# HpWang-whu/YOHO

Hardware: AMD Instinct MI355X
Metric: keypoints/sec (5000 kp x60 rot desc+YOHO-O) (higher is better)
Workload: dtype fp16x2 split (2^-22-accurate products, fp32 accumulate); 1 GPU

## Files before the change

yoho_amd/csrc/api.hip:

```cpp
#include "common.h"
#include <cstdarg>
#include <cstdio>
#include <cstring>
#include <cstdlib>
#include <cmath>
#include <vector>

namespace yoho {

static thread_local char g_err[512] = "";

void set_error(const char* fmt, ...) {
    va_list ap;
    va_start(ap, fmt);
    vsnprintf(g_err, sizeof(g_err), fmt, ap);
    va_end(ap);
}

void clear_error() { g_err[0] = 0; }

int hip_fail(hipError_t e, const char* what, const char* file, int line) {
    set_error("HIP error %d (%s) at %s:%d: %s", (int)e, hipGetErrorString(e), file, line, what);
    return YOHO_EHIP;
}
// ... 307 lines not shown
                            if (g < 0) g = ug[2 * u];
                            int tap = 2 * tp + h;
                            if (tap >= NTAP) tap = 2 * tp;
                            slab4[(cfg * 7 + tp) * 32 + u] |= (g < 0 ? 0 : (int)N[g * NTAP + tap]) << (8 * (2 * gs + h));
                        }
        }
        if ((rc = upload_slot_tables16(slab4.data(), unitg.data(), c->tabs)) || (rc = gconv16_init())) { delete c; return rc; }
    }
    c->gconv_mode = 4;
    c->partII_mode = 2;
    {
        auto is = [](const char* name, const char* val) { const char* e = std::getenv(name); return e && std::strcmp(e, val) == 0; };
        auto num = [](const char* name) { const char* e = std::getenv(name); return e ? std::atoi(e) : 0; };
        c->env.partII_tail_staged = is("YOHO_PARTII_TAIL", "staged");
        c->env.transfer_staged = is("YOHO_TRANSFER", "staged");
        c->env.xf_steal = !is("YOHO_XF_STEAL", "0");
        c->env.nn_splits = num("YOHO_NN_SPLITS");
        c->env.fcgf_f32 = is("YOHO_FCGF", "f32");
        c->env.fcgf_full_maps = is("YOHO_FCGF_MAPS", "full");
        c->env.fcgf_norm_staged = is("YOHO_FCGF_NORM", "staged");
        c->env.fcgf_heads_staged = is("YOHO_FCGF_HEADS", "staged");
        if (const char* e = std::getenv("YOHO_WS_LIMIT_MB")) c->env.ws_limit_mb = std::atoll(e);
        if (is("YOHO_PARTII_L1", "3")) c->env.partII_l1_variant = FG_TILE256_W8;
    }
    if (const char* m = std::getenv("YOHO_FCGF_CELLS")) c->fcgf_cell_sort = std::atoi(m);
    if (const char* m = std::getenv("YOHO_FCGF_SORT")) c->fcgf_parity_sort = std::strcmp(m, "0") == 0 ? 0 : 1;
    if (const char* m = std::getenv("YOHO_FCGF_COORDS")) c->fcgf_hash_coords = std::strcmp(m, "hash") == 0 ? 1 : 0;
    if (const char* m = std::getenv("YOHO_NN")) c->nn_prefilter = std::strcmp(m, "brute") == 0 ? 0 : 1;
    if (const char* m = std::getenv("YOHO_PARTII")) c->partII_mode = std::strcmp(m, "f32") == 0 ? 0 : (std::strcmp(m, "fp16x2") == 0 ? 2 : (std::strcmp(m, "cgemm") == 0 ? 3 : (std::strcmp(m, "cgemm8") == 0 ? 4 : 1)));
    if (const char* m = std::getenv("YOHO_PARTI_CHUNK")) {
        int ck = 0, ns = 1;
        if (std::sscanf(m, "%dx%d", &ck, &ns) >= 1 && ck >= 0 && (ns == 1 || ns == 2)) { c->partI_chunk = (ck + 255) / 256 * 256; c->partI_streams = ns; }
    }
    if (const char* m = std::getenv("YOHO_GCONV")) c->gconv_mode = std::strcmp(m, "f32") == 0 ? 0 : (std::strcmp(m, "bf16x3") == 0 ? 1 : (std::strcmp(m, "fp16x2") == 0 ? 3 : (std::strcmp(m, "fgemm") == 0 ? 4 : (std::strcmp(m, "fgemm256") == 0 ? 5 : (std::strcmp(m, "fgemm128") == 0 ? 6 : (std::strcmp(m, "fgemm8") == 0 ? 7 : 2))))));
    c->fb = new FourierBasis();
    if ((rc = build_fourier(N, P, *c->fb))) { delete c->fb; delete c; return rc; }
    {
        std::vector<float> fpad(2 * 64 * 64, 0.f);
        for (int s = 0; s < G; ++s)
            for (int g = 0; g < G; ++g) {
                fpad[s * 64 + g] = (float)c->fb->F[s * G + g];
                fpad[64 * 64 + g * 64 + s] = (float)c->fb->F[s * G + g];
            }
        if ((rc = upload(fpad.data(), fpad.size() * sizeof(float), (void**)&c->dFpad)) || (rc = gft_init()) || (rc = fgemm_init()) || (rc = gft16_init())) { delete c->fb; delete c; return rc; }
        std::vector<unsigned short> f16;
        build_gft16_frags(*c->fb, f16);
        if ((rc = upload(f16.data(), f16.size() * sizeof(unsigned short), &c->dF16))) { delete c->fb; delete c; return rc; }
        hipDeviceProp_t prop;
        if (hipGetDeviceProperties(&prop, device) == hipSuccess && prop.multiProcessorCount > 0) c->nCU = prop.multiProcessorCount;
    }
    HIPCHK(hipMalloc((void**)&c->d_rflag, 4 * sizeof(int)));
    HIPCHK(hipMemset(c->d_rflag, 0, 4 * sizeof(int)));
// ... 89 lines not shown
    if ((rc = build_layer(c->p2[2], w->res_out, 512, 256, NTAP, nullptr))) return rc;
    if ((rc = build_layer(c->p2[3], w->fc0, 256, 512, 1, &w->fc0_bn))) return rc;
    if ((rc = build_layer(c->p2[4], w->fc1, 512, 128, 1, &w->fc1_bn))) return rc;
    if ((rc = build_layer(c->p2[5], w->fc2, 128, 4, 1, nullptr))) return rc;
    for (auto& L : c->p2) L.tabs = &c->tabs;
    c->has_partII = true;
    return 0;
}

int yoho_set_gconv_mode(yoho_ctx* c, int mode) {
    if (!c || mode < 0 || mode > 7) { set_error("yoho_set_gconv_mode: mode must be 0 (fp32 MFMA), 1 (bf16x3 MFMA), 2 (group-Fourier fp32 MFMA), 3 (fp16x2 MFMA), 4 (group-Fourier irrep GEMMs, fp16x2 MFMA), 5 or 6 (4 with the other two GEMM blockings), 7 (4 with fp8 correction products)"); return YOHO_EINVAL; }
    c->gconv_mode = mode;
    return 0;
}

int yoho_set_partI_schedule(yoho_ctx* c, int chunk_kp, int streams) {
    if (!c || chunk_kp < 0 || streams < 1 || streams > 2) { set_error("yoho_set_partI_schedule: chunk_kp >= 0 and streams 1 or 2"); return YOHO_EINVAL; }
    c->partI_chunk = (chunk_kp + 255) / 256 * 256;
    c->partI_streams = streams;
    return 0;
}

int yoho_set_partII_mode(yoho_ctx* c, int mode) {
    if (!c || mode < 0 || mode > 4) { set_error("yoho_set_partII_mode: mode must be 0 (fp32 MFMA), 1 (bf16x3), 2 (fp16x2 MFMA, direct cone kernels), 3 (fp16x2, 13-element cone layer as an implicit GEMM) or 4 (3 with fp8 correction products)"); return YOHO_EINVAL; }
    c->partII_mode = mode;
    return 0;
}

int yoho_set_nn_prefilter(yoho_ctx* c, int enable) {
    if (!c) { set_error("yoho_set_nn_prefilter: null ctx"); return YOHO_EINVAL; }
    c->nn_prefilter = enable ? 1 : 0;
    return 0;
}

int yoho_set_fcgf_sort(yoho_ctx* c, int parity_sort, int cell_sort) {
    if (!c) { set_error("yoho_set_fcgf_sort: null ctx"); return YOHO_EINVAL; }
    c->fcgf_parity_sort = parity_sort ? 1 : 0;
    c->fcgf_hash_coords = (cell_sort >= 0 && (cell_sort & 4)) ? 1 : 0;
    cell_sort = cell_sort < 0 ? 0 : (cell_sort & 3);
    c->fcgf_cell_sort = cell_sort > 2 ? 2 : cell_sort;
    return 0;
}

int yoho_set_nn_grid(yoho_ctx* c, double cell) {
    if (!c || !(cell >= 0.0) || !std::isfinite(cell)) { set_error("yoho_set_nn_grid: cell must be a finite number >= 0 (0 = brute force)"); return YOHO_EINVAL; }
    c->nn_cell = cell;
    return 0;
// ... 353 lines not shown
                            inv_np ? inv_np + (size_t)b0 * F : nullptr, s);
        if (rc) return rc;
    }
    return 0;
}

int yoho_group_mean_np(yoho_ctx* c, const float* eqv, int B, float* out, void* stream) {
    if (!c || !eqv || !out || B < 0) { set_error("yoho_group_mean_np: bad argument"); return YOHO_EINVAL; }
    if (B == 0) return 0;
    YOHO_NEED_ALIGNED("yoho_group_mean_np", 15, eqv, out);
    HIPCHK(hipSetDevice(c->device));
    return launch_group_mean_np(eqv, B, out, (hipStream_t)stream);
}

static bool partII_fourier_head(const yoho_ctx* c) {
    return c->partII_mode >= 2 && c->p2[0].wpg;
}

static int partII_pass16(yoho_ctx* c, const float* s0, const float* s1, const float* s2, const float* s3, const int64_t* idx,
                         int M, float* quat, hipStream_t s, int npl, const int64_t* const* ridx = nullptr, int istride = 1) {
    const int nT16 = (M + 15) / 16, nT = (M + TILE - 1) / TILE;
    const size_t ch16 = (size_t)npl * 15360;
    const size_t n128 = (size_t)nT * 16, n256 = (size_t)nT * 32, n512 = (size_t)nT * 64, n32 = (size_t)nT * 4;
    const size_t szG = c->partII_mode >= 3 ? (size_t)((nT + 7) / 8) * c->cone_nslot * 8 * 32768 : 0;
    const size_t szX = (size_t)nT16 * 16 * ch16, szA0 = std::max((size_t)nT16 * 32 * ch16, szG);
    const size_t szA1p = npl == 2 ? (size_t)nT16 * 64 * ch16 : 0;
    int rc;
    int* rf = c->d_rflag + 1;
    if (ridx && !partII_fourier_head(c)) { set_error("indexed PartII needs the default (fp16x2, Fourier first layer) mode"); return YOHO_EINVAL; }
    const bool fourier_head = npl == 2 && partII_fourier_head(c);
    const int kppad = (M + 255) / 256 * 256;
    char *bX = nullptr, *bA0 = nullptr, *bA1p = nullptr, *bP = nullptr;
    float *bH0 = nullptr, *bA1 = nullptr, *bF = nullptr, *bF0 = nullptr, *bF1 = nullptr, *bQ = nullptr, *bC = nullptr;
    if ((rc = bind_ws(c, s, [&](Arena& ar) {
            bX = ar.take<char>(szX);
            bA0 = ar.take<char>(szA0);
            bA1p = ar.take<char>(szA1p);
            bH0 = ar.take<float>(n256 * CHUNK_FLOATS);
            bA1 = ar.take<float>(n512 * CHUNK_FLOATS);
            bF = ar.take<float>(n256 * CHUNK_FLOATS);
            bF0 = ar.take<float>(n512 * CHUNK_FLOATS);
            bF1 = ar.take<float>(n128 * CHUNK_FLOATS);
            bQ = ar.take<float>(n32 * CHUNK_FLOATS);
            if (fourier_head) {
                bP = ar.take<char>(fgemm_planes_bytes(kppad, 128));
                bC = ar.take<float>(n256 * CHUNK_FLOATS);
            }
        }))) return rc;
    if (fourier_head) {
        if ((rc = launch_head2(s0, s1, s2, s3, idx, c->dP, c->p2_init_bn_s, c->p2_init_bn_t, M, nT, bP, kppad, c->dF16, s, ridx, istride, rf))) return rc;
        if ((rc = launch_fgemm(c->p2[0], bP, kppad, nT, nullptr, bC, 0, s, rf, c->env.partII_l1_variant))) return rc;
        if (c->partII_mode >= 3 && c->p2[1].wcg && !c->env.partII_tail_staged && mlp_head_supported(c->p2[3], c->p2[4], c->p2[5])) {
            const int nslot = c->cone_nslot;
            unsigned* amax = nullptr;
            if (c->partII_mode == 4) {
                amax = c->d_amax + 8;
                HIPCHK(hipMemsetAsync(amax, 0, sizeof(unsigned), s));
            }
            if ((rc = launch_gft16_invg(bC, bH0, bA0, c->cone_slot_of, nslot, c->dF16, c->p2[0].bn_s, c->p2[0].bn_t, nT, 32, c->nCU, s, rf, amax))) return rc;
            if ((rc = launch_cgemm(c->p2[1], bA0, nslot, c->cone_slot, c->cone_outg, nT, nT16, bA1p, s, rf, amax))) return rc;
            int n0[NTAP];
            for (int k = 0; k < NTAP; ++k) n0[k] = c->hN[k];
            if ((rc = launch_cone1(c->p2[2], bA1p, nT, nT16, nullptr, nullptr, n0, s, bF0))) return rc;
            return launch_mlp_head(c->p2[3], c->p2[4], c->p2[5], nullptr, nT, M, quat, s, bF0, &c->p2[2], bH0);
        }
        if ((rc = launch_gft16_invp(bC, bH0, bA0, nT16, c->dF16, c->p2[0].bn_s, c->p2[0].bn_t, nT, 32, c->nCU, s, rf))) return rc;
    } else {
        if ((rc = launch_pack16_partII(s0, s1, s2, s3, idx, c->dP, c->p2_init_bn_s, c->p2_init_bn_t, M, nT16, bX, s, npl, rf))) return rc;
        if ((rc = launch_gconv16(c->p2[0], bX, nT16, nullptr, nullptr, bA0, EPI_RAW32 | EPI_ACT, s, 1, bH0, nullptr, npl, rf))) return rc;
    }
    if (npl == 2) {
        int n0[NTAP];
        for (int k = 0; k < NTAP; ++k) n0[k] = c->hN[k];
        if ((rc = launch_gconv16(c->p2[1], bA0, nT16, nullptr, nullptr, bA1p, EPI_ACT, s, 2, nullptr, nullptr, npl, rf))) return rc;
        if (!c->env.partII_tail_staged && mlp_head_supported(c->p2[3], c->p2[4], c->p2[5])) {
            if ((rc = launch_cone1(c->p2[2], bA1p, nT, nT16, nullptr, nullptr, n0, s, bF0))) return rc;
            return launch_mlp_head(c->p2[3], c->p2[4], c->p2[5], nullptr, nT, M, quat, s, bF0, &c->p2[2], bH0);
        }
        if ((rc = launch_cone1(c->p2[2], bA1p, nT, nT16, bH0, bF, n0, s))) return rc;
    } else {
        if ((rc = launch_gconv16(c->p2[1], bA0, nT16, nullptr, nullptr, nullptr, EPI_ACT32, s, 2, nullptr, bA1, npl))) return rc;
        if ((rc = launch_gconv(conv_args(c->p2[2], bA1, nT, bH0, bF, nullptr, true), -1, EPI_RES | EPI_RAW, s))) return rc;
    }
// ... 262 lines not shown
```

yoho_amd/csrc/common.h:

```cpp
#pragma once
#include <hip/hip_runtime.h>
#include <stdint.h>
#include <stddef.h>
#include <initializer_list>
#include "yoho_hip.h"
#include "arena.h"

namespace yoho {

constexpr int G = 60;
constexpr int NTAP = 13;
constexpr int F = 32;
constexpr int TILE = 32;
constexpr int SLAB_FLOATS = 2 * TILE * 4;
constexpr int CHUNK_FLOATS = G * SLAB_FLOATS;

void set_error(const char* fmt, ...);
void clear_error();
inline bool yoho_misaligned(std::initializer_list<const void*> ps, unsigned mask) {
    for (const void* p : ps) if ((reinterpret_cast<uintptr_t>(p) & mask) != 0) return true;
    return false;
}
#define YOHO_NEED_ALIGNED(fn, mask, ...)                                                                                  \
    do {                                                                                                                  \
// ... 90 lines not shown
int launch_finalize_partI(const float* y, const float* x, int B, float* eqv, float* inv, float* inv_np, int layout16, hipStream_t s,
                          const float* x1 = nullptr, int B0 = 0);
struct FourierBasis {
    double rho[5][60][25];
    double F[60 * 60];
    int n0[13];
};
int build_fourier(const uint8_t* N, const uint8_t* P, FourierBasis& fb);
}
#include <vector>
#include <cstdlib>
namespace yoho {
void pack_fourier_weights(const FourierBasis& fb, const float* W, int cin, int cout, int cout_pad, std::vector<float>& out);
int gft_init();
int fgemm_init();
size_t fgemm_planes_bytes(int kppad, int cin);
void fgemm_qinfo(int* qi);
void fgemm_plane_offsets(int kppad, int cin, long long* off);
int pack_fgemm_weights(const FourierBasis& fb, const float* W, int cin, int cout, std::vector<unsigned short>& out, float* descale,
                       std::vector<unsigned short>* out8 = nullptr);
int pack_cgemm_weights(const float* W, int cin, int cout, int ntaps, std::vector<unsigned short>& out, float* descale, std::vector<unsigned short>& out8);
int cgemm_init();
int launch_cgemm(const Layer& L, const char* Bstages, int nslot, const unsigned char* slot, const unsigned char* outg, int nT32, int nTiles16,
                 char* out, hipStream_t s, int* rflag, const unsigned* amax);
int launch_gft16_invg(const float* in, float* res0, char* planesG, const int* slot_of, int nslot, const void* Ffrag, const float* bn_s,
                      const float* bn_t, int nTiles, int C8, int nCU, hipStream_t s, int* rflag, unsigned* amax);
int launch_fgemm(const Layer& L, const char* Bplanes, int kppad, int nT32, const float* res, float* out, int flags, hipStream_t s,
                 int* rflag = nullptr, FGemmBlocking blocking = FG_TILE128, const unsigned* amax = nullptr);
void build_gft16_frags(const FourierBasis& fb, std::vector<unsigned short>& out);
int gconv_layer(yoho_ctx* c, const float* x, int B, int cin, int cout, const float* W, const float* bias, int transpose, float* y,
                hipStream_t s);
int bn_stats(const float* x, int B, int C, float* mean, float* var, hipStream_t s);
int bn_relu_apply(const float* x, int B, int C, const float* scale, const float* shift, float* y, hipStream_t s);
int bn_relu_apply_sub(const float* x, int B, int C, const float* mean, const float* scale, const float* beta, float* y, hipStream_t s);
int bn_relu_backward(const float* x, const float* y, const float* dy, int B, int C, const float* gamma, const float* mean, const float* rstd,
                     int batch_stats, float* dx, float* dgamma, float* dbeta, hipStream_t s);
int gconv_wgrad(yoho_ctx* c, const float* x, const float* dy, int B, int cin, int cout, float* dW, float* db, hipStream_t s);
struct FcgfNet;
int fcgf_load(FcgfNet** out, const yoho_fcgf_config* cfg, const float* const* t, int ntensors, bool f32_kernels);
void fcgf_free(FcgfNet* n);
int fcgf_forward(yoho_ctx* ctx, const FcgfNet* net, const int* coords0, int n0, const int* off_host, int nb, float* out, hipStream_t s);
int fcgf_voxelize(yoho_ctx* ctx, const double* pts, int n, const double* R_host, double voxel, int64_t* sel, int* coords, float* pts_sel,
                  int* count_host, hipStream_t s);
int fcgf_rotate_select(const double* pts, const double* R_host, const int64_t* sel, int m, float* out, hipStream_t s);
int fcgf_voxelize_batch(yoho_ctx* ctx, const double* pts, int n, const double* R_host, int nb, double voxel, int64_t* sel, int* coords,
                        float* pts_sel, int* counts_host, hipStream_t s);
int launch_cone1(const Layer& L, const char* X, int nTiles32, int nTiles16, const float* res, float* out, const int* n0, hipStream_t s, float* part = nullptr);
// ... 74 lines not shown
    bool on = false;
    std::vector<hipEvent_t> pool;
    size_t used = 0;
    struct Span { int cat; hipEvent_t a, b; };
    std::vector<Span> spans;
    int open_cat = -1;
    hipEvent_t open_ev = nullptr;
    double flops[NCAT] = {0};
    double launches[NCAT] = {0};
};

}

struct yoho_env_switches {
    bool partII_tail_staged = false;
    bool transfer_staged = false;
    bool xf_steal = true;
    int nn_splits = 0;
    bool fcgf_f32 = false;
    bool fcgf_full_maps = false;
    bool fcgf_norm_staged = false;
    bool fcgf_heads_staged = false;
    yoho::FGemmBlocking partII_l1_variant = yoho::FG_TILE128;
    long long ws_limit_mb = 0;
};

struct yoho_ctx {
    int device = 0;
    yoho_env_switches env;
    float* dR32 = nullptr;
    double* dR64 = nullptr;
    int* dN = nullptr;
    int* dP = nullptr;
    unsigned* dPq = nullptr;
    uint8_t hN[60 * 13];
    uint8_t hP[60 * 60];
    float hR[60 * 9];
    bool has_partI = false, has_partII = false;
    yoho::Layer p1[4];
    yoho::Layer p2[6];
    float *p2_init_bn_s = nullptr, *p2_init_bn_t = nullptr;
    int partII_mode = 2;
    int cone_nslot = 0;
    int cone_slot_of[60];
    unsigned char cone_slot[13 * 13];
    unsigned char cone_outg[13];
// ... 73 lines not shown
```

yoho_amd/csrc/gemmf2.hip:

```cpp
#include <hip/hip_runtime.h>
#include <cstdlib>
#include <cstring>
#include "common.h"
#include "gemmf.h"

namespace yoho {

constexpr int F2_BUF = 24576;
constexpr int F2_LDS = 3 * F2_BUF;
constexpr int F3_BUF = 32768;
constexpr int F3_LDS = 3 * F3_BUF;

struct Frags2 {
    uintx4 ah[4], al[4], bh[2], bl[2];
};

template <int LO, int R>
__device__ __forceinline__ void read_frag2(const char* pa, const char* pb, Frags2& f) {
    if constexpr (R < 4) f.al[R] = *reinterpret_cast<const uintx4*>(pa + 8192 + R * 512);
    else if constexpr (R < 6) f.bh[R - 4] = *reinterpret_cast<const uintx4*>(pb + (R - 4) * 512);
    else if constexpr (R < 10) f.ah[R - 6] = *reinterpret_cast<const uintx4*>(pa + (R - 6) * 512);
    else f.bl[R - 10] = *reinterpret_cast<const uintx4*>(pb + LO + (R - 10) * 512);
}
template <int LO>
// ... 115 lines not shown
    constexpr std::false_type nodma;
    while (s + 4 < KT) {
        run(dma, P, Q);
        run(dma, Q, P);
    }
    if (KT >= 4) {
        run(dma, P, Q);
        run(nodma, Q, P);
    }
    run(nodma, P, Q);
    step(nodma, Q, P, smem + cur + lane_a, smem + cur + lane_b, nullptr, nullptr, nullptr);
}

template <int BUF, typename Dma>
__device__ __forceinline__ void ring_pipelined_idle(int KT, Dma&& dma) {
    __builtin_amdgcn_s_barrier();
    for (int s = 0; s + 1 < KT; ++s) {
        if (s + 3 < KT) dma(s + 3, (s % 3) * BUF);
        asm volatile("s_waitcnt vmcnt(0)" ::: "memory");
        __builtin_amdgcn_s_barrier();
    }
}

__global__ __launch_bounds__(256, 2) void fgemm2_kernel(FGemmArgs a, int flags) {
    extern __shared__ __attribute__((aligned(16))) char smem[];
    const int tid = threadIdx.x, lane = tid & 63;
    const int w = __builtin_amdgcn_readfirstlane(tid >> 6);
    int t = 0, local = 0, r = 0;
    if (!fg2_map(a, blockIdx.x & 7, blockIdx.x >> 3, (flags & F2_MIX) == 0, t, local, r)) return;
    const int d = a.dim[t];
    const int MT = a.MT[t], KS = d * a.cin / 32, KT = 2 * KS;
    const int nh = local & 1, pair = local >> 1;
    const int cg = pair / MT, mtile = pair - cg * MT;
    const int ntile = r + 8 * cg;
    const char* Ag = a.A + a.a_off[t] + (size_t)mtile * KS * FG_STAGE;
    const char* Bg = a.B + a.b_off[t] + (size_t)ntile * KS * FG_STAGE + nh * 2048;
    const int wm = w >> 1, wn = w & 1;
    const Dma2 dm(w, lane);
    const int lane_a = (lane >> 5) * 4096 + (wm * 128 + (lane & 31)) * 16;
    const int lane_b = 16384 + (lane >> 5) * 2048 + (wn * 64 + (lane & 31)) * 16;

    floatx16 acc[4][2];
    zero_acc(acc);
    auto dma = [&](int st, int buf) { dma_step(dm, Ag + step_off(st), Bg + step_off(st), smem + buf); };
    ring_prologue<F2_BUF>(KT, dma);
    const int row0 = mtile * 256 + wm * 128, colbase = ntile * 256 + nh * 128 + wn * 64;
    const bool rows_live = row0 < d * a.cout;
    const int jidx = colbase / a.kppad, kp0 = colbase - jidx * a.kppad, qbase = a.qbase[t];
    if ((flags & EPI_RES) && rows_live) residual_start(acc, row0, kp0, jidx, d, qbase, a.res, a.descale, a.cout, a.nT32, lane);
    asm volatile("s_waitcnt vmcnt(0)" ::: "memory");
    __builtin_amdgcn_s_barrier();
    if (!rows_live) return ring_pipelined_idle<F2_BUF>(KT, dma);

    Frags2 P;
    read_frags2<Dma2::LO>(smem + lane_a, smem + lane_b, P);
    ring_pipelined<F2_BUF, 6>(smem, Ag, Bg, KT, lane_a, lane_b, P,
        [&](auto dmac, const Frags2& f, Frags2& nf, const char* ra, const char* rb, const char* srcA, const char* srcB, char* buf) {
            step2<decltype(dmac)::value>(dm, f, acc, ra, rb, nf, srcA, srcB, buf);
        });
    coef_epilogue(acc, row0, kp0, jidx, d, qbase, a.out, a.bias, a.descale, a.cout, a.nT32, a.rflag, lane, flags);
}

struct Wave3 {
    int wm, wn, nh, lane_a, lane_b;
    Dma3 dm;
    __device__ __forceinline__ Wave3(int w8, int lane) : wm((w8 & 3) >> 1), wn(w8 & 1), nh(w8 >> 2), dm(w8, lane) {
        lane_a = (lane >> 5) * 4096 + (wm * 128 + (lane & 31)) * 16;
        lane_b = 16384 + (lane >> 5) * 4096 + (nh * 128 + wn * 64 + (lane & 31)) * 16;
    }
};

__global__ __launch_bounds__(512, 2) void fgemm3_kernel(FGemmArgs a, int flags) {
    extern __shared__ __attribute__((aligned(16))) char smem[];
    const int tid = threadIdx.x, lane = tid & 63;
    const Wave3 wv(__builtin_amdgcn_readfirstlane(tid >> 6), lane);
    int t = 0, local = 0, r = 0;
    if (!fg3_map(a, blockIdx.x & 7, blockIdx.x >> 3, t, local, r)) return;
    const int d = a.dim[t];
    const int MT = a.MT[t], KS = d * a.cin / 32, KT = 2 * KS;
    const int cg = local / MT, mtile = local - cg * MT;
    const int ntile = r + 8 * cg;
    const char* Ag = a.A + a.a_off[t] + (size_t)mtile * KS * FG_STAGE;
    const char* Bg = a.B + a.b_off[t] + (size_t)ntile * KS * FG_STAGE;

    floatx16 acc[4][2];
    zero_acc(acc);
    auto dma = [&](int st, int buf) { dma_step(wv.dm, Ag + step_off(st), Bg + step_off(st), smem + buf); };
    ring_prologue<F3_BUF>(KT, dma);
    const int row0 = mtile * 256 + wv.wm * 128, colbase = ntile * 256 + wv.nh * 128 + wv.wn * 64;
    const bool rows_live = row0 < d * a.cout;
    const int jidx = colbase / a.kppad, kp0 = colbase - jidx * a.kppad, qbase = a.qbase[t];
// ... 48 lines not shown
__device__ __forceinline__ void step3c(const Frags2& f, floatx16 (&acc)[4][2], Frags8& c8, const C8Scales& sc) {
#pragma unroll
    for (int i = 0; i < 4; ++i)
#pragma unroll
        for (int j = 0; j < 2; ++j) acc[i][j] = mfma_h(f.ah[i], f.bh[j], acc[i][j]);
#pragma unroll
    for (int i = 0; i < 4; ++i)
#pragma unroll
        for (int e = 0; e < 4; ++e) c8.a[i][4 * PAR + e] = (int)f.al[i][e];
#pragma unroll
    for (int j = 0; j < 2; ++j) {
        const Int2 l = frag_to_fp8(f.bl[j], sc.bl), h = frag_to_fp8(f.bh[j], sc.bh);
        c8.b[j][4 * PAR] = l.x; c8.b[j][4 * PAR + 1] = l.y; c8.b[j][4 * PAR + 2] = h.x; c8.b[j][4 * PAR + 3] = h.y;
    }
    if constexpr (PAR == 1) {
#pragma unroll
        for (int i = 0; i < 4; ++i)
#pragma unroll
            for (int j = 0; j < 2; ++j)
                acc[i][j] = __builtin_amdgcn_mfma_scale_f32_32x32x64_f8f6f4(c8.a[i], c8.b[j], acc[i][j], 0, 0, 0, 127 + 2 - 11, 0, sc.mfma_b);
    }
}

template <bool FP8, typename BSrc>
__device__ __forceinline__ void ring_plain(floatx16 (&acc)[4][2], char* smem, const Wave3& wv, const char* Ag, BSrc&& bsrc, int KT, bool rows_live,
                                           const C8Scales& sc) {
    Frags8 c8;
    if constexpr (FP8) {
#pragma unroll
        for (int i = 0; i < 4; ++i)
#pragma unroll
            for (int e = 0; e < 8; ++e) c8.a[i][e] = 0;
#pragma unroll
        for (int j = 0; j < 2; ++j)
#pragma unroll
            for (int e = 0; e < 8; ++e) c8.b[j][e] = 0;
    }
    int cur = 0, stg = 2 * F3_BUF;
    int s = 0;
    auto stage = [&] {
        const int s2 = s + 2 < KT ? s + 2 : KT - 1;
        dma_step(wv.dm, uniform_ptr(Ag + step_off(s2)), uniform_ptr(bsrc(s2)), smem + stg);
    };
    auto rotate = [&] { stg = cur; cur = cur == 2 * F3_BUF ? 0 : cur + F3_BUF; ++s; };
    auto one_step = [&](auto parity) {
        asm volatile("s_waitcnt vmcnt(4) lgkmcnt(0)" ::: "memory");
        __builtin_amdgcn_s_barrier();
        __builtin_amdgcn_sched_barrier(0);
        stage();
        Frags2 f;
        read_frags2<Dma3::LO>(smem + cur + wv.lane_a, smem + cur + wv.lane_b, f);
        if constexpr (FP8) step3c<decltype(parity)::value>(f, acc, c8, sc);
        else {
#pragma unroll
            for (int i = 0; i < 4; ++i)
#pragma unroll
                for (int j = 0; j < 2; ++j) acc[i][j] = mfma_h(f.al[i], f.bh[j], acc[i][j]);
#pragma unroll
            for (int i = 0; i < 4; ++i)
#pragma unroll
                for (int j = 0; j < 2; ++j) acc[i][j] = mfma_h(f.ah[i], f.bl[j], acc[i][j]);
#pragma unroll
            for (int i = 0; i < 4; ++i)
#pragma unroll
                for (int j = 0; j < 2; ++j) acc[i][j] = mfma_h(f.ah[i], f.bh[j], acc[i][j]);
        }
        rotate();
    };
    if (rows_live) {
        for (int it = 0; it < KT; it += 2) {
            one_step(std::integral_constant<int, 0>{});
            one_step(std::integral_constant<int, 1>{});
        }
    } else {
        for (int it = 0; it < KT; ++it) {
            asm volatile("s_waitcnt vmcnt(4) lgkmcnt(0)" ::: "memory");
            __builtin_amdgcn_s_barrier();
            stage();
            rotate();
        }
    }
    asm volatile("s_waitcnt vmcnt(0)" ::: "memory");
}

__global__ __launch_bounds__(512, 2) void fgemm3c_kernel(FGemmArgs a, int flags) {
    extern __shared__ __attribute__((aligned(16))) char smem[];
    const int tid = threadIdx.x, lane = tid & 63;
    const Wave3 wv(__builtin_amdgcn_readfirstlane(tid >> 6), lane);
    int t = 0, local = 0, r = 0;
    if (!fg3_map(a, blockIdx.x & 7, blockIdx.x >> 3, t, local, r)) return;
    const int d = a.dim[t];
    const int MT = a.MT[t], KS = d * a.cin / 32, KT = 2 * KS;
    const int cg = local / MT, mtile = local - cg * MT;
    const int ntile = r + 8 * cg;
    const char* Ag = a.A + a.a_off[t] + (size_t)mtile * KS * FG_STAGE;
    const char* Bg = a.B + a.b_off[t] + (size_t)ntile * KS * FG_STAGE;

    floatx16 acc[4][2];
    zero_acc(acc);
// ... 17 lines not shown
    const float* bias;
    const float* bn_s;
    const float* bn_t;
    char* out;
    int NTm, MT, KSt, ntap, nj, nslot, c8out, nT32, nTiles16;
    float descale;
    int* rflag;
    const unsigned* amax;
    unsigned char slot[13 * 13];
    unsigned char outg[16];
};

__device__ __forceinline__ void cg_split_pair(float x0, float x1, unsigned& hi, unsigned& lo) {
    typedef float f2 __attribute__((ext_vector_type(2)));
    f2 x;
    x.x = x0; x.y = x1;
    const halfx2 h = __builtin_convertvector(x, halfx2);
    const f2 r = x - __builtin_convertvector(h, f2);
    const halfx2 l = __builtin_convertvector(r, halfx2);
    __builtin_memcpy(&hi, &h, 4);
    __builtin_memcpy(&lo, &l, 4);
}

template <bool FP8>
__global__ __launch_bounds__(512, 2) void cgemm_kernel(CGemmArgs a) {
    extern __shared__ __attribute__((aligned(16))) char smem[];
    __shared__ int tapoff[16];
    const int tid = threadIdx.x, lane = tid & 63;
    const Wave3 wv(__builtin_amdgcn_readfirstlane(tid >> 6), lane);
    const int xcd = blockIdx.x & 7, slot_ = blockIdx.x >> 3;
    const int ct = xcd + 8 * (slot_ / a.MT), mtile = slot_ % a.MT;
    if (ct >= a.nj * a.NTm) return;
    const int j = ct / a.NTm, mt = ct - j * a.NTm;
    const int SPT = 2 * a.KSt;
    const int KT = a.ntap * SPT;
    if (tid < 16) tapoff[tid] = tid < a.ntap ? (int)a.slot[j * 13 + tid] : 0;
    const char* Ag = a.A + (size_t)mtile * (KT / 2) * FG_STAGE;
    const char* Bt = a.B + (size_t)mt * a.nslot * a.KSt * FG_STAGE;
    __syncthreads();
    auto bsrc = [&](int s) -> const char* {
        const int tap = s / SPT, within = s - tap * SPT;
        const int sl = __builtin_amdgcn_readfirstlane(tapoff[tap]);
        return Bt + (size_t)sl * a.KSt * FG_STAGE + step_off(within);
    };

    floatx16 acc[4][2];
    zero_acc(acc);
    C8Scales sc;
    if constexpr (FP8) sc = C8Scales(a.amax);
    dma_step(wv.dm, Ag, uniform_ptr(bsrc(0)), smem);
    dma_step(wv.dm, Ag + step_off(1), uniform_ptr(bsrc(1)), smem + F3_BUF);
    asm volatile("s_waitcnt vmcnt(0)" ::: "memory");
    __builtin_amdgcn_s_barrier();

    ring_plain<FP8>(acc, smem, wv, Ag, bsrc, KT, true, sc);

    const int half = lane >> 5, c32 = lane & 31;
    const int g = a.outg[j];
    unsigned top = 0u;
#pragma unroll
    for (int bi = 0; bi < 2; ++bi) {
        const int m = mt * 256 + wv.nh * 128 + wv.wn * 64 + bi * 32 + c32;
        if ((m >> 5) >= a.nT32 || (m >> 4) >= a.nTiles16) continue;
#pragma unroll
        for (int ai = 0; ai < 4; ++ai) {
#pragma unroll
            for (int q4 = 0; q4 < 4; ++q4) {
                const int o = mtile * 256 + wv.wm * 128 + ai * 32 + q4 * 8 + half * 4;
                const floatx4 b4 = *reinterpret_cast<const floatx4*>(a.bias + o);
                const floatx4 s4 = *reinterpret_cast<const floatx4*>(a.bn_s + o);
                const floatx4 t4 = *reinterpret_cast<const floatx4*>(a.bn_t + o);
                float y[4];
#pragma unroll
                for (int e = 0; e < 4; ++e) {
                    const float v = acc[ai][bi][4 * q4 + e] * a.descale + b4[e];
                    y[e] = fmaxf(v * s4[e] + t4[e], 0.f) * H2_ASCALE;
                    top = max(top, __float_as_uint(y[e]) & 0x7FFFFFFFu);
                }
                unsigned h0, l0, h1, l1;
                cg_split_pair(y[0], y[1], h0, l0);
                cg_split_pair(y[2], y[3], h1, l1);
                char* dst = a.out + (((size_t)(m >> 4) * a.c8out + (o >> 3)) * 2) * 15360 + g * 256 + (m & 15) * 16 + half * 8;
                *reinterpret_cast<uint2*>(dst) = uint2{h0, h1};
                *reinterpret_cast<uint2*>(dst + 15360) = uint2{l0, l1};
            }
        }
    }
    note_range_bits(a.rflag, top, FP16_MAX);
}

int cgemm_init() {
    HIPCHK(hipFuncSetAttribute(reinterpret_cast<const void*>(&cgemm_kernel<true>), hipFuncAttributeMaxDynamicSharedMemorySize, F3_LDS));
    HIPCHK(hipFuncSetAttribute(reinterpret_cast<const void*>(&cgemm_kernel<false>), hipFuncAttributeMaxDynamicSharedMemorySize, F3_LDS));
    return 0;
}

int launch_cgemm(const Layer& L, const char* Bstages, int nslot, const unsigned char* slot, const unsigned char* outg, int nT32, int nTiles16,
                 char* out, hipStream_t s, int* rflag, const unsigned* amax) {
    const bool fp8 = amax != nullptr;
    if (!(fp8 ? L.wcg8 : L.wcg) || L.cin % 32 || L.cout % 256) { set_error("cgemm: needs the cone-GEMM weight pack, cin %% 32 == 0, cout %% 256 == 0"); return YOHO_EINVAL; }
    if (nT32 == 0) return 0;
    CGemmArgs a;
    a.A = reinterpret_cast<const char*>(fp8 ? L.wcg8 : L.wcg); a.B = Bstages; a.bias = L.bias; a.bn_s = L.bn_s; a.bn_t = L.bn_t; a.out = out;
    a.NTm = (nT32 + 7) / 8; a.MT = L.cout / 256; a.KSt = L.cin / 32; a.ntap = 13; a.nj = 13; a.nslot = nslot; a.c8out = L.cout / 8;
    a.nT32 = nT32; a.nTiles16 = nTiles16; a.descale = L.wcg_descale; a.rflag = rflag; a.amax = amax;
    std::memcpy(a.slot, slot, 169);
    std::memset(a.outg, 0, 16);
    std::memcpy(a.outg, outg, 13);
    const int CT = a.nj * a.NTm;
    const int grid = 8 * ((CT + 7) / 8) * a.MT;
    if (fp8) hipLaunchKernelGGL(cgemm_kernel<true>, dim3(grid), dim3(512), F3_LDS, s, a);
    else hipLaunchKernelGGL(cgemm_kernel<false>, dim3(grid), dim3(512), F3_LDS, s, a);
    HIPCHK(hipGetLastError());
    return 0;
}

struct Frags3s {
    uintx4 ah[5], al[5], bh, bl;
};

template <int R>
__device__ __forceinline__ void read_frag3s(const char* pa, const char* pb, Frags3s& f) {
    if constexpr (R < 5) f.al[R] = *reinterpret_cast<const uintx4*>(pa + 8192 + R * 512);
    else if constexpr (R == 5) f.bh = *reinterpret_cast<const uintx4*>(pb);
    else if constexpr (R < 11) f.ah[R - 6] = *reinterpret_cast<const uintx4*>(pa + (R - 6) * 512);
    else f.bl = *reinterpret_cast<const uintx4*>(pb + 8192);
}

template <bool DMA, int D>
__device__ __forceinline__ void step3s(const Frags3s& f, floatx16 (&acc)[5][1], const char* ra, const char* rb, Frags3s& nf,
                                       const char* srcA, const char* srcB, char* dmabuf, const Dma3& dm) {
    sfor<0, 5>([&](auto gc) {
        constexpr int g = decltype(gc)::value;
        if constexpr (g < D) acc[g][0] = mfma_h(f.al[g], f.bh, acc[g][0]);
        if constexpr (g < D) read_frag3s<g>(ra, rb, nf);
// ... 106 lines not shown
```

yoho_amd/hip.py:

```python
import ctypes as C
import os
import sys
import threading
import warnings
import numpy as np
import torch

from . import tables as _tables
from . import weights as _weights

_LIB_PATH = os.path.join(os.path.dirname(os.path.abspath(__file__)), "lib",
                         "libyoho_hip_exp.so" if os.environ.get("YOHO_LIB") == "exp" else "libyoho_hip.so")
_lib = None

SYMBOLS = [
    "yoho_last_error", "yoho_version", "yoho_ctx_create", "yoho_ctx_destroy", "yoho_load_partI",
    "yoho_load_partII", "yoho_partI_forward", "yoho_partI_forward_pair", "yoho_group_mean_np", "yoho_nn_search", "yoho_mutual_nn",
    "yoho_gconv_layer", "yoho_load_fcgf", "yoho_fcgf_voxelize", "yoho_fcgf_forward", "yoho_fcgf_forward_batch", "yoho_fcgf_voxelize_rotated", "yoho_rotate_select",
    "yoho_des2r", "yoho_des2r_indexed", "yoho_partII_forward", "yoho_partII_forward_indexed", "yoho_hyp_from_quat", "yoho_o_score", "yoho_c_ransac",
    "yoho_group_gather", "yoho_set_profiling", "yoho_get_kernel_ms", "yoho_set_gconv_mode", "yoho_set_partII_mode", "yoho_set_nn_grid",
    "yoho_range_status", "yoho_c_ransac_device", "yoho_group_scatter", "yoho_set_nn_prefilter", "yoho_set_fcgf_sort", "yoho_fcgf_voxelize_rotated_batch", "yoho_gconv_wgrad", "yoho_bn_stats", "yoho_bn_relu_apply", "yoho_bn_relu_apply_sub", "yoho_bn_relu_backward", "yoho_set_partI_schedule", "yoho_clock_probe", "yoho_group_transfer_batch",
    "yoho_register_pair", "yoho_vote_order", "yoho_c_draw_np", "yoho_phase_profile", "yoho_phase_read", "yoho_poison_scratch",
]
KNN_SYMBOLS = ["yoho_knn_search"]
# ... 168 lines not shown
    pos = C.c_int(int(st[2]))
    prob = np.ascontiguousarray(prob, dtype=np.float64)
    start = np.ascontiguousarray(bucket_start, dtype=np.int64)
    members = np.ascontiguousarray(bucket_members, dtype=np.int64)
    if prob.shape != (60,) or start.shape != (61,) or members.ndim != 1 or int(start[-1]) > members.shape[0]:
        raise ValueError("c_draw_np: prob (60,), bucket_start (61,), bucket_members (>= bucket_start[60],)")
    tri = np.empty((max(int(max_iter), 0), 3), dtype=np.int64)
    n, draws = C.c_int(0), C.c_int(0)
    rc = lib.yoho_c_draw_np(key.ctypes.data_as(C.c_void_p), C.byref(pos), prob.ctypes.data_as(C.c_void_p), start.ctypes.data_as(C.c_void_p),
                            members.ctypes.data_as(C.c_void_p), int(max_iter), tri.ctypes.data_as(C.c_void_p), C.byref(n), C.byref(draws))
    if rc != 0:
        raise YohoError(f"libyoho_hip error {rc}: {lib.yoho_last_error().decode()}", rc)
    src.set_state((st[0], key, pos.value) + tuple(st[3:]))
    return tri[:n.value], draws.value


class YohoError(RuntimeError):
    def __init__(self, msg, code=0):
        super().__init__(msg)
        self.code = code


GCONV_MODES = {"f32": 0, "bf16x3": 1, "fourier": 2, "fp16x2": 3, "fgemm": 4, "fgemm256": 5, "fgemm128": 6, "fgemm8": 7}
PARTII_MODES = {"f32": 0, "bf16x3": 1, "fp16x2": 2, "cgemm": 3, "cgemm8": 4}
FP16_PARTII_MODES = ("fp16x2", "cgemm", "cgemm8")
FP16_GCONV_MODES = ("fp16x2", "fgemm", "fgemm256", "fgemm128", "fgemm8")
MAX_PAIR_KEYPOINTS = 16384


def _check(rc):
    if rc != 0:
        raise YohoError(f"libyoho_hip error {rc}: {_lib.yoho_last_error().decode()}", rc)


def _np_ptr(a):
    return a.ctypes.data_as(C.c_void_p)


def _stream():
    return C.c_void_p(torch.cuda.current_stream().cuda_stream)


def _dev(t, dtype, name):
    if not (isinstance(t, torch.Tensor) and t.is_cuda):
        raise TypeError(f"{name}: expected a CUDA/HIP tensor")
    if t.dtype != dtype:
        raise TypeError(f"{name}: expected dtype {dtype}, got {t.dtype}")
    if not t.is_contiguous():
# ... 867 lines not shown
```

Before: 1.902 million keypoints/s.

## Route default PartII mode through cone GEMM with 128-wide pipelined tiles

Mode 2, the default, now runs the 13-element cone layer as an implicit GEMM; before, only modes 3 and 4 did. The old direct cone kernels move to a new mode 5. The cone GEMM gains a 128-column tile variant by default: 256-thread workgroups, two per output tile, using a deeper ring-pipelined tap loop that prefetches fragments. This aims to replace the direct cone kernels and to raise occupancy and latency hiding, at the cost of more workgroups and duplicated A-tile loads.

```diff
diff --git a/yoho_amd/csrc/api.hip b/yoho_amd/csrc/api.hip
--- a/yoho_amd/csrc/api.hip
+++ b/yoho_amd/csrc/api.hip
@@ -353,12 +353,13 @@
         c->env.fcgf_heads_staged = is("YOHO_FCGF_HEADS", "staged");
         if (const char* e = std::getenv("YOHO_WS_LIMIT_MB")) c->env.ws_limit_mb = std::atoll(e);
         if (is("YOHO_PARTII_L1", "3")) c->env.partII_l1_variant = FG_TILE256_W8;
+        if (is("YOHO_PARTII_CONE", "256")) c->env.partII_cone_tile = 256;
     }
     if (const char* m = std::getenv("YOHO_FCGF_CELLS")) c->fcgf_cell_sort = std::atoi(m);
     if (const char* m = std::getenv("YOHO_FCGF_SORT")) c->fcgf_parity_sort = std::strcmp(m, "0") == 0 ? 0 : 1;
     if (const char* m = std::getenv("YOHO_FCGF_COORDS")) c->fcgf_hash_coords = std::strcmp(m, "hash") == 0 ? 1 : 0;
     if (const char* m = std::getenv("YOHO_NN")) c->nn_prefilter = std::strcmp(m, "brute") == 0 ? 0 : 1;
-    if (const char* m = std::getenv("YOHO_PARTII")) c->partII_mode = std::strcmp(m, "f32") == 0 ? 0 : (std::strcmp(m, "fp16x2") == 0 ? 2 : (std::strcmp(m, "cgemm") == 0 ? 3 : (std::strcmp(m, "cgemm8") == 0 ? 4 : 1)));
+    if (const char* m = std::getenv("YOHO_PARTII")) c->partII_mode = std::strcmp(m, "f32") == 0 ? 0 : (std::strcmp(m, "fp16x2") == 0 ? 2 : (std::strcmp(m, "cgemm") == 0 ? 3 : (std::strcmp(m, "cgemm8") == 0 ? 4 : (std::strcmp(m, "fp16x2d") == 0 ? 5 : 1))));
     if (const char* m = std::getenv("YOHO_PARTI_CHUNK")) {
         int ck = 0, ns = 1;
         if (std::sscanf(m, "%dx%d", &ck, &ns) >= 1 && ck >= 0 && (ns == 1 || ns == 2)) { c->partI_chunk = (ck + 255) / 256 * 256; c->partI_streams = ns; }
@@ -494,7 +495,7 @@
 }
 
 int yoho_set_partII_mode(yoho_ctx* c, int mode) {
-    if (!c || mode < 0 || mode > 4) { set_error("yoho_set_partII_mode: mode must be 0 (fp32 MFMA), 1 (bf16x3), 2 (fp16x2 MFMA, direct cone kernels), 3 (fp16x2, 13-element cone layer as an implicit GEMM) or 4 (3 with fp8 correction products)"); return YOHO_EINVAL; }
+    if (!c || mode < 0 || mode > 5) { set_error("yoho_set_partII_mode: mode must be 0 (fp32 MFMA), 1 (bf16x3), 2 (fp16x2 MFMA, 13-element cone layer as an implicit GEMM), 3 (the same), 4 (2 with fp8 correction products) or 5 (fp16x2 MFMA, direct cone kernels)"); return YOHO_EINVAL; }
     c->partII_mode = mode;
     return 0;
 }
@@ -894,7 +895,9 @@
     const int nT16 = (M + 15) / 16, nT = (M + TILE - 1) / TILE;
     const size_t ch16 = (size_t)npl * 15360;
     const size_t n128 = (size_t)nT * 16, n256 = (size_t)nT * 32, n512 = (size_t)nT * 64, n32 = (size_t)nT * 4;
-    const size_t szG = c->partII_mode >= 3 ? (size_t)((nT + 7) / 8) * c->cone_nslot * 8 * 32768 : 0;
+    const bool cone_gemm = npl == 2 && c->partII_mode >= 2 && c->partII_mode <= 4 && partII_fourier_head(c) && c->p2[1].wcg &&
+                           !c->env.partII_tail_staged && mlp_head_supported(c->p2[3], c->p2[4], c->p2[5]);
+    const size_t szG = cone_gemm ? (size_t)((nT + 7) / 8) * c->cone_nslot * 8 * 32768 : 0;
     const size_t szX = (size_t)nT16 * 16 * ch16, szA0 = std::max((size_t)nT16 * 32 * ch16, szG);
     const size_t szA1p = npl == 2 ? (size_t)nT16 * 64 * ch16 : 0;
     int rc;
@@ -922,7 +925,7 @@
     if (fourier_head) {
         if ((rc = launch_head2(s0, s1, s2, s3, idx, c->dP, c->p2_init_bn_s, c->p2_init_bn_t, M, nT, bP, kppad, c->dF16, s, ridx, istride, rf))) return rc;
         if ((rc = launch_fgemm(c->p2[0], bP, kppad, nT, nullptr, bC, 0, s, rf, c->env.partII_l1_variant))) return rc;
-        if (c->partII_mode >= 3 && c->p2[1].wcg && !c->env.partII_tail_staged && mlp_head_supported(c->p2[3], c->p2[4], c->p2[5])) {
+        if (cone_gemm) {
             const int nslot = c->cone_nslot;
             unsigned* amax = nullptr;
             if (c->partII_mode == 4) {
@@ -930,7 +933,7 @@
                 HIPCHK(hipMemsetAsync(amax, 0, sizeof(unsigned), s));
             }
             if ((rc = launch_gft16_invg(bC, bH0, bA0, c->cone_slot_of, nslot, c->dF16, c->p2[0].bn_s, c->p2[0].bn_t, nT, 32, c->nCU, s, rf, amax))) return rc;
-            if ((rc = launch_cgemm(c->p2[1], bA0, nslot, c->cone_slot, c->cone_outg, nT, nT16, bA1p, s, rf, amax))) return rc;
+            if ((rc = launch_cgemm(c->p2[1], bA0, nslot, c->cone_slot, c->cone_outg, nT, nT16, bA1p, s, rf, amax, c->env.partII_cone_tile))) return rc;
             int n0[NTAP];
             for (int k = 0; k < NTAP; ++k) n0[k] = c->hN[k];
             if ((rc = launch_cone1(c->p2[2], bA1p, nT, nT16, nullptr, nullptr, n0, s, bF0))) return rc;
diff --git a/yoho_amd/csrc/common.h b/yoho_amd/csrc/common.h
--- a/yoho_amd/csrc/common.h
+++ b/yoho_amd/csrc/common.h
@@ -136,7 +136,7 @@
 int pack_cgemm_weights(const float* W, int cin, int cout, int ntaps, std::vector<unsigned short>& out, float* descale, std::vector<unsigned short>& out8);
 int cgemm_init();
 int launch_cgemm(const Layer& L, const char* Bstages, int nslot, const unsigned char* slot, const unsigned char* outg, int nT32, int nTiles16,
-                 char* out, hipStream_t s, int* rflag, const unsigned* amax);
+                 char* out, hipStream_t s, int* rflag, const unsigned* amax, int tile);
 int launch_gft16_invg(const float* in, float* res0, char* planesG, const int* slot_of, int nslot, const void* Ffrag, const float* bn_s,
                       const float* bn_t, int nTiles, int C8, int nCU, hipStream_t s, int* rflag, unsigned* amax);
 int launch_fgemm(const Layer& L, const char* Bplanes, int kppad, int nT32, const float* res, float* out, int flags, hipStream_t s,
@@ -257,6 +257,7 @@
     bool fcgf_norm_staged = false;
     bool fcgf_heads_staged = false;
     yoho::FGemmBlocking partII_l1_variant = yoho::FG_TILE128;
+    int partII_cone_tile = 128;
     long long ws_limit_mb = 0;
 };
 
diff --git a/yoho_amd/csrc/gemmf2.hip b/yoho_amd/csrc/gemmf2.hip
--- a/yoho_amd/csrc/gemmf2.hip
+++ b/yoho_amd/csrc/gemmf2.hip
@@ -161,6 +161,38 @@
     }
 }
 
+template <int BUF, int INFLIGHT, typename F, typename BSrc, typename Step>
+__device__ __forceinline__ void ring_pipelined_taps(char* smem, const char* Ag, BSrc&& bsrc, int KT, int lane_a, int lane_b, F& P, Step&& step) {
+    F Q;
+    asm volatile("s_waitcnt lgkmcnt(0)" ::: "memory");
+    __builtin_amdgcn_s_barrier();
+    __builtin_amdgcn_sched_barrier(0);
+    int cur = 0, nxt = BUF;
+    int s = 0;
+    auto run = [&](auto dma, const F& f, F& nf) {
+        if constexpr (decltype(dma)::value) {
+            step(dma, f, nf, smem + nxt + lane_a, smem + nxt + lane_b, uniform_ptr(Ag + step_off(s + 3)), uniform_ptr(bsrc(s + 3)), smem + cur);
+            asm volatile("s_waitcnt vmcnt(%0) lgkmcnt(0)" ::"n"(INFLIGHT) : "memory");
+        } else {
+            step(dma, f, nf, smem + nxt + lane_a, smem + nxt + lane_b, nullptr, nullptr, nullptr);
+            asm volatile("s_waitcnt vmcnt(0) lgkmcnt(0)" ::: "memory");
+        }
+        __builtin_amdgcn_s_barrier();
+        __builtin_amdgcn_sched_barrier(0);
+        cur = nxt; nxt = nxt == 2 * BUF ? 0 : nxt + BUF; ++s;
+    };
+    constexpr std::true_type dma;
+    constexpr std::false_type nodma;
+    while (s + 4 < KT) {
+        run(dma, P, Q);
+        run(dma, Q, P);
+    }
+    run(dma, P, Q);
+    run(nodma, Q, P);
+    run(nodma, P, Q);
+    step(nodma, Q, P, smem + cur + lane_a, smem + cur + lane_b, nullptr, nullptr, nullptr);
+}
+
 __global__ __launch_bounds__(256, 2) void fgemm2_kernel(FGemmArgs a, int flags) {
     extern __shared__ __attribute__((aligned(16))) char smem[];
     const int tid = threadIdx.x, lane = tid & 63;
@@ -201,11 +233,21 @@
 }
 
 struct Wave3 {
+    static constexpr int BUF = F3_BUF, THREADS = 512, WG_PER_TILE = 1;
     int wm, wn, nh, lane_a, lane_b;
     Dma3 dm;
     __device__ __forceinline__ Wave3(int w8, int lane) : wm((w8 & 3) >> 1), wn(w8 & 1), nh(w8 >> 2), dm(w8, lane) {
         lane_a = (lane >> 5) * 4096 + (wm * 128 + (lane & 31)) * 16;
         lane_b = 16384 + (lane >> 5) * 4096 + (nh * 128 + wn * 64 + (lane & 31)) * 16;
+    }
+};
+struct Wave2 {
+    static constexpr int BUF = F2_BUF, THREADS = 256, WG_PER_TILE = 2;
+    int wm, wn, lane_a, lane_b;
+    Dma2 dm;
+    __device__ __forceinline__ Wave2(int w, int lane) : wm(w >> 1), wn(w & 1), dm(w, lane) {
+        lane_a = (lane >> 5) * 4096 + (wm * 128 + (lane & 31)) * 16;
+        lane_b = 16384 + (lane >> 5) * 2048 + (wn * 64 + (lane & 31)) * 16;
     }
 };
 
@@ -300,9 +342,11 @@
     }
 }
 
-template <bool FP8, typename BSrc>
-__device__ __forceinline__ void ring_plain(floatx16 (&acc)[4][2], char* smem, const Wave3& wv, const char* Ag, BSrc&& bsrc, int KT, bool rows_live,
+template <bool FP8, typename Wave, typename BSrc>
+__device__ __forceinline__ void ring_plain(floatx16 (&acc)[4][2], char* smem, const Wave& wv, const char* Ag, BSrc&& bsrc, int KT, bool rows_live,
                                            const C8Scales& sc) {
+    using Dma = decltype(Wave::dm);
+    constexpr int BUF = Wave::BUF;
     Frags8 c8;
     if constexpr (FP8) {
 #pragma unroll
@@ -314,20 +358,20 @@
 #pragma unroll
             for (int e = 0; e < 8; ++e) c8.b[j][e] = 0;
     }
-    int cur = 0, stg = 2 * F3_BUF;
+    int cur = 0, stg = 2 * BUF;
     int s = 0;
     auto stage = [&] {
         const int s2 = s + 2 < KT ? s + 2 : KT - 1;
         dma_step(wv.dm, uniform_ptr(Ag + step_off(s2)), uniform_ptr(bsrc(s2)), smem + stg);
     };
-    auto rotate = [&] { stg = cur; cur = cur == 2 * F3_BUF ? 0 : cur + F3_BUF; ++s; };
+    auto rotate = [&] { stg = cur; cur = cur == 2 * BUF ? 0 : cur + BUF; ++s; };
     auto one_step = [&](auto parity) {
-        asm volatile("s_waitcnt vmcnt(4) lgkmcnt(0)" ::: "memory");
+        asm volatile("s_waitcnt vmcnt(%0) lgkmcnt(0)" ::"n"(Dma::NP) : "memory");
         __builtin_amdgcn_s_barrier();
         __builtin_amdgcn_sched_barrier(0);
         stage();
         Frags2 f;
-        read_frags2<Dma3::LO>(smem + cur + wv.lane_a, smem + cur + wv.lane_b, f);
+        read_frags2<Dma::LO>(smem + cur + wv.lane_a, smem + cur + wv.lane_b, f);
         if constexpr (FP8) step3c<decltype(parity)::value>(f, acc, c8, sc);
         else {
 #pragma unroll
@@ -352,7 +396,7 @@
         }
     } else {
         for (int it = 0; it < KT; ++it) {
-            asm volatile("s_waitcnt vmcnt(4) lgkmcnt(0)" ::: "memory");
+            asm volatile("s_waitcnt vmcnt(%0) lgkmcnt(0)" ::"n"(Dma::NP) : "memory");
             __builtin_amdgcn_s_barrier();
             stage();
             rotate();
@@ -416,21 +460,27 @@
     __builtin_memcpy(&lo, &l, 4);
 }
 
-template <bool FP8>
-__global__ __launch_bounds__(512, 2) void cgemm_kernel(CGemmArgs a) {
+template <bool FP8, typename Wave>
+__global__ __launch_bounds__(Wave::THREADS, 2) void cgemm_kernel(CGemmArgs a) {
     extern __shared__ __attribute__((aligned(16))) char smem[];
     __shared__ int tapoff[16];
     const int tid = threadIdx.x, lane = tid & 63;
-    const Wave3 wv(__builtin_amdgcn_readfirstlane(tid >> 6), lane);
-    const int xcd = blockIdx.x & 7, slot_ = blockIdx.x >> 3;
+    const Wave wv(__builtin_amdgcn_readfirstlane(tid >> 6), lane);
+    const int xcd = blockIdx.x & 7;
+    int slot_ = blockIdx.x >> 3, nh;
+    if constexpr (Wave::WG_PER_TILE == 2) { nh = slot_ & 1; slot_ >>= 1; }
+    else nh = wv.nh;
     const int ct = xcd + 8 * (slot_ / a.MT), mtile = slot_ % a.MT;
     if (ct >= a.nj * a.NTm) return;
     const int j = ct / a.NTm, mt = ct - j * a.NTm;
+    if constexpr (Wave::WG_PER_TILE == 2) {
+        if (mt * 8 + nh * 4 >= a.nT32) return;
+    }
     const int SPT = 2 * a.KSt;
     const int KT = a.ntap * SPT;
     if (tid < 16) tapoff[tid] = tid < a.ntap ? (int)a.slot[j * 13 + tid] : 0;
     const char* Ag = a.A + (size_t)mtile * (KT / 2) * FG_STAGE;
-    const char* Bt = a.B + (size_t)mt * a.nslot * a.KSt * FG_STAGE;
+    const char* Bt = a.B + (size_t)mt * a.nslot * a.KSt * FG_STAGE + (Wave::WG_PER_TILE == 2 ? nh * 2048 : 0);
     __syncthreads();
     auto bsrc = [&](int s) -> const char* {
         const int tap = s / SPT, within = s - tap * SPT;
@@ -440,21 +490,34 @@
 
     floatx16 acc[4][2];
     zero_acc(acc);
-    C8Scales sc;
-    if constexpr (FP8) sc = C8Scales(a.amax);
-    dma_step(wv.dm, Ag, uniform_ptr(bsrc(0)), smem);
-    dma_step(wv.dm, Ag + step_off(1), uniform_ptr(bsrc(1)), smem + F3_BUF);
-    asm volatile("s_waitcnt vmcnt(0)" ::: "memory");
-    __builtin_amdgcn_s_barrier();
-
-    ring_plain<FP8>(acc, smem, wv, Ag, bsrc, KT, true, sc);
+    if constexpr (!FP8 && Wave::WG_PER_TILE == 2) {
+        using Dma = decltype(Wave::dm);
+        ring_prologue<Wave::BUF>(KT, [&](int st, int buf) { dma_step(wv.dm, uniform_ptr(Ag + step_off(st)), uniform_ptr(bsrc(st)), smem + buf); });
+        asm volatile("s_waitcnt vmcnt(0)" ::: "memory");
+        __builtin_amdgcn_s_barrier();
+        Frags2 P;
+        read_frags2<Dma::LO>(smem + wv.lane_a, smem + wv.lane_b, P);
+        ring_pipelined_taps<Wave::BUF, Dma::NP>(smem, Ag, bsrc, KT, wv.lane_a, wv.lane_b, P,
+            [&](auto dmac, const Frags2& f, Frags2& nf, const char* ra, const char* rb, const char* srcA, const char* srcB, char* buf) {
+                step2<decltype(dmac)::value>(wv.dm, f, acc, ra, rb, nf, srcA, srcB, buf);
+            });
+    } else {
+        C8Scales sc;
+        if constexpr (FP8) sc = C8Scales(a.amax);
+        dma_step(wv.dm, Ag, uniform_ptr(bsrc(0)), smem);
+        dma_step(wv.dm, Ag + step_off(1), uniform_ptr(bsrc(1)), smem + Wave::BUF);
+        asm volatile("s_waitcnt vmcnt(0)" ::: "memory");
+        __builtin_amdgcn_s_barrier();
+
+        ring_plain<FP8>(acc, smem, wv, Ag, bsrc, KT, true, sc);
+    }
 
     const int half = lane >> 5, c32 = lane & 31;
     const int g = a.outg[j];
     unsigned top = 0u;
 #pragma unroll
     for (int bi = 0; bi < 2; ++bi) {
-        const int m = mt * 256 + wv.nh * 128 + wv.wn * 64 + bi * 32 + c32;
+        const int m = mt * 256 + nh * 128 + wv.wn * 64 + bi * 32 + c32;
         if ((m >> 5) >= a.nT32 || (m >> 4) >= a.nTiles16) continue;
 #pragma unroll
         for (int ai = 0; ai < 4; ++ai) {
@@ -484,14 +547,17 @@
 }
 
 int cgemm_init() {
-    HIPCHK(hipFuncSetAttribute(reinterpret_cast<const void*>(&cgemm_kernel<true>), hipFuncAttributeMaxDynamicSharedMemorySize, F3_LDS));
-    HIPCHK(hipFuncSetAttribute(reinterpret_cast<const void*>(&cgemm_kernel<false>), hipFuncAttributeMaxDynamicSharedMemorySize, F3_LDS));
+    HIPCHK(hipFuncSetAttribute(reinterpret_cast<const void*>(&cgemm_kernel<true, Wave3>), hipFuncAttributeMaxDynamicSharedMemorySize, F3_LDS));
+    HIPCHK(hipFuncSetAttribute(reinterpret_cast<const void*>(&cgemm_kernel<false, Wave3>), hipFuncAttributeMaxDynamicSharedMemorySize, F3_LDS));
+    HIPCHK(hipFuncSetAttribute(reinterpret_cast<const void*>(&cgemm_kernel<true, Wave2>), hipFuncAttributeMaxDynamicSharedMemorySize, F2_LDS));
+    HIPCHK(hipFuncSetAttribute(reinterpret_cast<const void*>(&cgemm_kernel<false, Wave2>), hipFuncAttributeMaxDynamicSharedMemorySize, F2_LDS));
     return 0;
 }
 
 int launch_cgemm(const Layer& L, const char* Bstages, int nslot, const unsigned char* slot, const unsigned char* outg, int nT32, int nTiles16,
-                 char* out, hipStream_t s, int* rflag, const unsigned* amax) {
+                 char* out, hipStream_t s, int* rflag, const unsigned* amax, int tile) {
     const bool fp8 = amax != nullptr;
+    if (tile != 128 && tile != 256) { set_error("cgemm: tile must be 128 or 256"); return YOHO_EINVAL; }
     if (!(fp8 ? L.wcg8 : L.wcg) || L.cin % 32 || L.cout % 256) { set_error("cgemm: needs the cone-GEMM weight pack, cin %% 32 == 0, cout %% 256 == 0"); return YOHO_EINVAL; }
     if (nT32 == 0) return 0;
     CGemmArgs a;
@@ -503,8 +569,11 @@
     std::memcpy(a.outg, outg, 13);
     const int CT = a.nj * a.NTm;
     const int grid = 8 * ((CT + 7) / 8) * a.MT;
-    if (fp8) hipLaunchKernelGGL(cgemm_kernel<true>, dim3(grid), dim3(512), F3_LDS, s, a);
-    else hipLaunchKernelGGL(cgemm_kernel<false>, dim3(grid), dim3(512), F3_LDS, s, a);
+    if (tile == 128) {
+        if (fp8) hipLaunchKernelGGL((cgemm_kernel<true, Wave2>), dim3(2 * grid), dim3(Wave2::THREADS), F2_LDS, s, a);
+        else hipLaunchKernelGGL((cgemm_kernel<false, Wave2>), dim3(2 * grid), dim3(Wave2::THREADS), F2_LDS, s, a);
+    } else if (fp8) hipLaunchKernelGGL((cgemm_kernel<true, Wave3>), dim3(grid), dim3(Wave3::THREADS), F3_LDS, s, a);
+    else hipLaunchKernelGGL((cgemm_kernel<false, Wave3>), dim3(grid), dim3(Wave3::THREADS), F3_LDS, s, a);
     HIPCHK(hipGetLastError());
     return 0;
 }
diff --git a/yoho_amd/hip.py b/yoho_amd/hip.py
--- a/yoho_amd/hip.py
+++ b/yoho_amd/hip.py
@@ -214,8 +214,8 @@
 
 
 GCONV_MODES = {"f32": 0, "bf16x3": 1, "fourier": 2, "fp16x2": 3, "fgemm": 4, "fgemm256": 5, "fgemm128": 6, "fgemm8": 7}
-PARTII_MODES = {"f32": 0, "bf16x3": 1, "fp16x2": 2, "cgemm": 3, "cgemm8": 4}
-FP16_PARTII_MODES = ("fp16x2", "cgemm", "cgemm8")
+PARTII_MODES = {"f32": 0, "bf16x3": 1, "fp16x2": 2, "cgemm": 3, "cgemm8": 4, "fp16x2d": 5}
+FP16_PARTII_MODES = ("fp16x2", "cgemm", "cgemm8", "fp16x2d")
 FP16_GCONV_MODES = ("fp16x2", "fgemm", "fgemm256", "fgemm128", "fgemm8")
 MAX_PAIR_KEYPOINTS = 16384
 
```

New measurement: 1.915 million keypoints/s, median of 6. No clear change (+0.7%).
